# yanyan-li/PlanarSLAM

Measured on NVIDIA H100. Metric: rgbd_frames_per_sec_640x480, higher is better.
Workload: dtype u8/f64

## Files before the change

planarslam_b200/csrc/lsd_kernels.cuh:

```cuda
#pragma once
#include <cuda_runtime.h>

#include <cfloat>
#include <cstdint>

#include "lsd_detsincos.h"
#include "lsd_rectenum.h"
#include "pslam_internal.h"

namespace pslam {

struct LsdGeom {
    int w, h;
    int W, H;
    int refine;
    int seg_cap;
    int cand_cap;
    int r2r_staged;
    int rect_enum;
    int min_reg_size;
    double rho, prec, p, log_nt, density_th, log_eps;
    const double* lgamma_tab;
};
#define LSD_LGAMMA_N 8192

#define LSD_ANG_UNDEF 0x7f800000u
#define LSD_ANG_USED 0x80000000u

#define LSD_PI 3.14159265358979323846
#define LSD_DEG2RAD (LSD_PI / 180)
#define LSD_3_2_PI ((3 * LSD_PI) / 2)
#define LSD_2PI (2 * LSD_PI)
#define LSD_LN10 2.30258509299404568402

__device__ __forceinline__ float lsd_fast_atan2_deg(float y, float x) {
    const float p1 = 0.9997878412794807f * (float)(180 / 3.14159265358979323846);
    const float p3 = -0.3258083974640975f * (float)(180 / 3.14159265358979323846);
    const float p5 = 0.1555786518463281f * (float)(180 / 3.14159265358979323846);
    const float p7 = -0.04432655554792128f * (float)(180 / 3.14159265358979323846);
    const float ax = fabsf(x), ay = fabsf(y);
    const bool wide = ax >= ay;
    const float num = wide ? ay : ax, den = __fadd_rn(wide ? ax : ay, (float)DBL_EPSILON);
    const float c = __fdiv_rn(num, den);
    const float c2 = __fmul_rn(c, c);
    float a = __fmul_rn(__fadd_rn(__fmul_rn(__fadd_rn(__fmul_rn(__fadd_rn(__fmul_rn(p7, c2), p5), c2), p3), c2), p1), c);
    if (!wide) a = __fsub_rn(90.f, a);
    if (x < 0) a = __fsub_rn(180.f, a);
    if (y < 0) a = __fsub_rn(360.f, a);
    return a;
}
__device__ __forceinline__ double lsd_angle(int gx, int gy) { return (double)lsd_fast_atan2_deg((float)gx, (float)(-gy)) * LSD_DEG2RAD; }
__device__ __forceinline__ double lsd_norm(int gx, int gy) { return sqrt((double)(gx * gx + gy * gy) / 4.0); }

template <int V>
__device__ __noinline__ void lsd_sincos(double x, double& s, double& c) { lsd_sincos_body(x, s, c); }

#define LSD_TW 64
#define LSD_TH 16
#define LSD_SW 88
#define LSD_SH 28
__global__ void __launch_bounds__(256) k_lsd_blur_scale(LsdGeom g, const uint8_t* __restrict__ gray, const int16_t* __restrict__ ix,
                                                        const int16_t* __restrict__ ax, const int16_t* __restrict__ iy, const int16_t* __restrict__ ay,
                                                        uint8_t* __restrict__ scaled) {
    __shared__ uint8_t s_src[LSD_SH][LSD_SW];
    __shared__ uint16_t s_h[LSD_SH][LSD_SW];
    __shared__ uint8_t s_b[LSD_SH][LSD_SW];
    const int frame = blockIdx.z, X0 = blockIdx.x * LSD_TW, Y0 = blockIdx.y * LSD_TH;
    const int X1 = min(X0 + LSD_TW, g.W) - 1, Y1 = min(Y0 + LSD_TH, g.H) - 1;
    const int bx0 = ix[X0], bx1 = min(ix[X1] + 1, g.w - 1), by0 = iy[Y0], by1 = min(iy[Y1] + 1, g.h - 1);
    const int sx0 = bx0 - 2, sy0 = by0 - 2, sw = bx1 - bx0 + 5, sh = by1 - by0 + 5;
    const uint8_t* src = gray + (size_t)frame * g.w * g.h;
// ... 61 lines not shown

__global__ void __launch_bounds__(256) k_lsd_gradient4(LsdGeom g, const uint8_t* __restrict__ scaled, const float2* __restrict__ cs_lut,
                                                       uint32_t* __restrict__ ang, float2* __restrict__ cs_out, uint32_t* __restrict__ gxy, int32_t* __restrict__ smax) {
    const int frame = blockIdx.z;
    const int W4 = g.W >> 2;
    const int xq = blockIdx.x * 64 + (threadIdx.x & 63), y = blockIdx.y * 4 + (threadIdx.x >> 6);
    const bool inside = xq < W4 && y < g.H;
    const uint8_t* s = scaled + (size_t)frame * g.W * g.H;
    uint32_t a_w[4] = {LSD_ANG_UNDEF, LSD_ANG_UNDEF, LSD_ANG_UNDEF, LSD_ANG_UNDEF}, g_w[4] = {0, 0, 0, 0};
    float2 cs[4];
#pragma unroll
    for (int i = 0; i < 4; ++i) cs[i] = make_float2(0.f, 0.f);
    int sq = 0;
    if (inside && y < g.H - 1) {
        const int x = xq * 4;
        const uint32_t* r0 = reinterpret_cast<const uint32_t*>(s + (size_t)y * g.W + x);
        const uint32_t* r1 = reinterpret_cast<const uint32_t*>(s + (size_t)(y + 1) * g.W + x);
        const uint32_t w0 = r0[0], w1 = r1[0];
        const bool more = x + 4 < g.W;
        const uint32_t n0 = more ? (uint32_t)s[(size_t)y * g.W + x + 4] : 0u, n1 = more ? (uint32_t)s[(size_t)(y + 1) * g.W + x + 4] : 0u;
        const uint32_t e0 = __funnelshift_r(w0, n0, 8), e1 = __funnelshift_r(w1, n1, 8);
#pragma unroll
        for (int i = 0; i < 4; ++i) {
            if (x + i >= g.W - 1) continue;
            const int pa = (w0 >> (8 * i)) & 255, pb = (e0 >> (8 * i)) & 255, pc = (w1 >> (8 * i)) & 255, pd = (e1 >> (8 * i)) & 255;
            const int DA = pd - pa, BC = pb - pc;
            const int gx = DA + BC, gy = DA - BC;
            g_w[i] = ((uint32_t)gx & 0xffffu) | ((uint32_t)gy << 16);
            if (lsd_norm(gx, gy) > g.rho) {
                sq = max(sq, gx * gx + gy * gy); a_w[i] = __float_as_uint(lsd_fast_atan2_deg((float)gx, (float)(-gy)));
                cs[i] = __ldg(cs_lut + (gx + 510) * 1021 + (gy + 510));
            }
        }
    }
    if (inside) {
        const size_t o = (size_t)frame * g.W * g.H + (size_t)y * g.W + (size_t)xq * 4;
        *reinterpret_cast<uint4*>(ang + o) = make_uint4(a_w[0], a_w[1], a_w[2], a_w[3]);
        *reinterpret_cast<uint4*>(gxy + o) = make_uint4(g_w[0], g_w[1], g_w[2], g_w[3]);
        float4* co = reinterpret_cast<float4*>(cs_out + o);
        co[0] = make_float4(cs[0].x, cs[0].y, cs[1].x, cs[1].y);
        co[1] = make_float4(cs[2].x, cs[2].y, cs[3].x, cs[3].y);
    }
    for (int o = 16; o; o >>= 1) sq = max(sq, __shfl_xor_sync(0xffffffffu, sq, o));
    if ((threadIdx.x & 31) == 0 && sq > 0) atomicMax(&smax[frame], sq);
}

struct LsdRect { double x1, y1, x2, y2, width, x, y, theta, dx, dy, prec, p; };

#define LSD_RING 64
struct LsdFrame {
    uint32_t* ang;
    const float2* cs; const uint32_t* gxy;
    uint32_t* reg; uint32_t* order;
    uint32_t* ring;
    int W, H;
};
__device__ __forceinline__ bool lsd_word_used(uint32_t w) { return (w & LSD_ANG_USED) != 0; }
__device__ __forceinline__ bool lsd_word_defined(uint32_t w) { return (w & 0x7fffffffu) < LSD_ANG_UNDEF; }
__device__ __forceinline__ float lsd_word_deg(uint32_t w) { return __uint_as_float(w & 0x7fffffffu); }
__device__ __forceinline__ double lsd_word_angle(uint32_t w) { return (double)lsd_word_deg(w) * LSD_DEG2RAD; }
__device__ __forceinline__ double lsd_pix_norm(const LsdFrame& F, int x, int y) {
    const uint32_t v = __ldg(F.gxy + (size_t)y * F.W + x);
    return lsd_norm((int)(short)(v & 0xffff), (int)(short)(v >> 16));
}

__device__ __forceinline__ bool lsd_aligned_angle(double a, double theta, double prec) {
    double n_theta = theta - a;
    if (n_theta < 0) n_theta = -n_theta;
    if (n_theta > LSD_3_2_PI) {
        n_theta -= LSD_2PI;
        if (n_theta < 0) n_theta = -n_theta;
    }
    return n_theta <= prec;
}

__device__ __forceinline__ double lsd_angle_diff_signed(double a, double b) {
    double diff = a - b;
    while (diff <= -LSD_PI) diff += LSD_2PI;
    while (diff > LSD_PI) diff -= LSD_2PI;
    return diff;
}
__device__ __forceinline__ bool lsd_double_equal(double a, double b) {
    if (a == b) return true;
    const double abs_diff = fabs(a - b), aa = fabs(a), bb = fabs(b);
    double abs_max = (aa > bb) ? aa : bb;
    if (abs_max < DBL_MIN) abs_max = DBL_MIN;
    return (abs_diff / abs_max) <= (100.0 * DBL_EPSILON);
}
__device__ __forceinline__ double lsd_dist_sq(double x1, double y1, double x2, double y2) { return (x2 - x1) * (x2 - x1) + (y2 - y1) * (y2 - y1); }

__device__ __forceinline__ uint32_t lsd_reg_read(const LsdFrame& F, int idx, int size) {
    return size - idx <= LSD_RING ? F.ring[idx & (LSD_RING - 1)] : F.reg[idx];
}
template <int V>
__device__ __noinline__ int lsd_region_grow(const LsdFrame& F, const LsdGeom& g, uint32_t seed, double prec, double& reg_angle_out) {
    const int lane = threadIdx.x & 31;
    const int q = lane >> 3, k8 = lane & 7;
    const int kk = k8 + (k8 >= 4);
    const int dyl = kk / 3 - 1, dxl = kk % 3 - 1;
    const int sx = seed & 0xffff, sy = seed >> 16;
    const uint32_t ws = F.ang[(size_t)sy * F.W + sx];
    double reg_angle = lsd_word_angle(ws);
    const double seed_angle = reg_angle;
    float sumdx = 0.f, sumdy = 0.f;
    if (lane == 0) { F.reg[0] = seed; F.ring[0] = seed; F.ang[(size_t)sy * F.W + sx] = ws | LSD_ANG_USED; }
    __syncwarp();
    int size = 1, i = 0;
    bool have_next = false;
    uint32_t np_next = 0xffffffffu, w_next = LSD_ANG_UNDEF;
    while (true) {
        const int navail = min(4, size - i);
        uint32_t npix, w;
        if (have_next) { npix = np_next; w = w_next; }
        else {
            npix = 0xffffffffu; w = LSD_ANG_UNDEF;
            if (q < navail) {
                const uint32_t pp = lsd_reg_read(F, i + q, size);
                const int nx = (int)(pp & 0xffff) + dxl, ny = (int)(pp >> 16) + dyl;
                if (nx >= 0 && ny >= 0 && nx < F.W && ny < F.H) { w = F.ang[(size_t)ny * F.W + nx]; npix = (uint32_t)nx | ((uint32_t)ny << 16); }
            }
        }
        have_next = size - i >= 8;
        np_next = 0xffffffffu; w_next = LSD_ANG_UNDEF;
        if (have_next) {
            const uint32_t pp = lsd_reg_read(F, i + 4 + q, size);
            const int nx = (int)(pp & 0xffff) + dxl, ny = (int)(pp >> 16) + dyl;
            if (nx >= 0 && ny >= 0 && nx < F.W && ny < F.H) { w_next = F.ang[(size_t)ny * F.W + nx]; np_next = (uint32_t)nx | ((uint32_t)ny << 16); }
        }
        bool cand = lsd_word_defined(w) && !lsd_word_used(w);
        const double a_n = lsd_word_angle(w);
        float2 csv = make_float2(0.f, 0.f);
        bool have_cs = cand && lsd_aligned_angle(a_n, reg_angle, prec);
        if (have_cs) csv = __ldg(F.cs + (size_t)(npix >> 16) * F.W + (npix & 0xffff));
        int last = -1;
        while (true) {
            const bool al = cand && lane > last && lsd_aligned_angle(a_n, reg_angle, prec);
            const unsigned m = __ballot_sync(0xffffffffu, al);
            if (!m) break;
            const int j = __ffs(m) - 1;
            if (lane == j) {
                if (!have_cs) { csv = __ldg(F.cs + (size_t)(npix >> 16) * F.W + (npix & 0xffff)); have_cs = true; }
                F.ang[(size_t)(npix >> 16) * F.W + (npix & 0xffff)] = w | LSD_ANG_USED;
                F.reg[size] = npix; F.ring[size & (LSD_RING - 1)] = npix;
            }
            const float cj = __shfl_sync(0xffffffffu, csv.x, j), sj = __shfl_sync(0xffffffffu, csv.y, j);
            const uint32_t np = __shfl_sync(0xffffffffu, npix, j);
            if (size == 1) { double sn0, cs0; lsd_sincos<V>(seed_angle, sn0, cs0); sumdx = (float)cs0; sumdy = (float)sn0; }
            sumdx = __fadd_rn(sumdx, cj);
            sumdy = __fadd_rn(sumdy, sj);
            reg_angle = (double)lsd_fast_atan2_deg(sumdy, sumdx) * LSD_DEG2RAD;
            if (npix == np) cand = false;
            if (np_next == np) w_next |= LSD_ANG_USED;
            ++size;
            last = j;
        }
        __syncwarp();
        i += navail;
        if (i >= size) break;
    }
    reg_angle_out = reg_angle;
    return size;
}

template <int V>
__device__ __noinline__ void lsd_region2rect_shfl(const LsdFrame& F, int size, double reg_angle, double prec, double p, LsdRect& rec) {
    const int lane = threadIdx.x & 31;
    double x = 0, y = 0, sum = 0;
    for (int base = 0; base < size; base += 32) {
        int mx = 0, my = 0; double mw = 0;
        if (base + lane < size) {
            const uint32_t pp = F.reg[base + lane];
            mx = pp & 0xffff; my = pp >> 16;
            mw = lsd_pix_norm(F, mx, my);
        }
        const int cnt = min(32, size - base);
        for (int t = 0; t < cnt; ++t) {
            const double w = __shfl_sync(0xffffffffu, mw, t);
            const int px = __shfl_sync(0xffffffffu, mx, t), py = __shfl_sync(0xffffffffu, my, t);
            x += (double)px * w;
            y += (double)py * w;
            sum += w;
        }
    }
    x /= sum;
    y /= sum;
    double Ixx = 0.0, Iyy = 0.0, Ixy = 0.0;
    for (int base = 0; base < size; base += 32) {
        int mx = 0, my = 0; double mw = 0;
        if (base + lane < size) {
            const uint32_t pp = F.reg[base + lane];
            mx = pp & 0xffff; my = pp >> 16;
            mw = lsd_pix_norm(F, mx, my);
        }
        const int cnt = min(32, size - base);
        for (int t = 0; t < cnt; ++t) {
            const double w = __shfl_sync(0xffffffffu, mw, t);
            const double ddx = (double)__shfl_sync(0xffffffffu, mx, t) - x, ddy = (double)__shfl_sync(0xffffffffu, my, t) - y;
            Ixx += ddy * ddy * w;
            Iyy += ddx * ddx * w;
            Ixy -= ddx * ddy * w;
        }
    }
    const double lambda = 0.5 * (Ixx + Iyy - sqrt((Ixx - Iyy) * (Ixx - Iyy) + 4.0 * Ixy * Ixy));
    double theta = (fabs(Ixx) > fabs(Iyy)) ? (double)lsd_fast_atan2_deg((float)(lambda - Ixx), (float)Ixy) : (double)lsd_fast_atan2_deg((float)Ixy, (float)(lambda - Iyy));
    theta *= LSD_DEG2RAD;
    if (fabs(lsd_angle_diff_signed(theta, reg_angle)) > prec) theta += LSD_PI;
    double dx, dy;
    lsd_sincos<V>(theta, dy, dx);
    double l_min = 0, l_max = 0, w_min = 0, w_max = 0;
    for (int base = 0; base < size; base += 32) {
        int mx = 0, my = 0;
        if (base + lane < size) { const uint32_t pp = F.reg[base + lane]; mx = pp & 0xffff; my = pp >> 16; }
        const int cnt = min(32, size - base);
        for (int t = 0; t < cnt; ++t) {
            const double regdx = (double)__shfl_sync(0xffffffffu, mx, t) - x, regdy = (double)__shfl_sync(0xffffffffu, my, t) - y;
            const double l = regdx * dx + regdy * dy;
            const double w = -regdx * dy + regdy * dx;
            if (l > l_max) l_max = l; else if (l < l_min) l_min = l;
            if (w > w_max) w_max = w; else if (w < w_min) w_min = w;
        }
    }
    rec.x1 = x + l_min * dx; rec.y1 = y + l_min * dy;
    rec.x2 = x + l_max * dx; rec.y2 = y + l_max * dy;
    rec.width = w_max - w_min;
    rec.x = x; rec.y = y; rec.theta = theta; rec.dx = dx; rec.dy = dy; rec.prec = prec; rec.p = p;
    if (rec.width < 1.0) rec.width = 1.0;
}

template <int V>
__device__ __noinline__ void lsd_region2rect(const LsdFrame& F, const LsdGeom& g, int size, double reg_angle, double prec, double p, LsdRect& rec) {
    if (!g.r2r_staged) { lsd_region2rect_shfl<V>(F, size, reg_angle, prec, p, rec); return; }
    __shared__ double s_stage[96];
    const int lane = threadIdx.x & 31;
    const double* const mine = s_stage + 32 * (lane < 3 ? lane : 2);
    double acc = 0;
    for (int base = 0; base < size; base += 32) {
        if (base + lane < size) {
            const uint32_t pp = F.reg[base + lane];
            const int mx = pp & 0xffff, my = pp >> 16;
            const double mw = lsd_pix_norm(F, mx, my);
            s_stage[lane] = (double)mx * mw; s_stage[32 + lane] = (double)my * mw; s_stage[64 + lane] = mw;
        }
        __syncwarp();
        const int cnt = min(32, size - base);
        for (int t = 0; t < cnt; ++t) acc += mine[t];
        __syncwarp();
    }
    const double sum = __shfl_sync(0xffffffffu, acc, 2);
    const double x = __shfl_sync(0xffffffffu, acc, 0) / sum, y = __shfl_sync(0xffffffffu, acc, 1) / sum;
    acc = 0;
    for (int base = 0; base < size; base += 32) {
        if (base + lane < size) {
            const uint32_t pp = F.reg[base + lane];
            const int mx = pp & 0xffff, my = pp >> 16;
            const double mw = lsd_pix_norm(F, mx, my);
            const double ddx = (double)mx - x, ddy = (double)my - y;
            s_stage[lane] = ddy * ddy * mw; s_stage[32 + lane] = ddx * ddx * mw; s_stage[64 + lane] = -(ddx * ddy * mw);
        }
        __syncwarp();
        const int cnt = min(32, size - base);
        for (int t = 0; t < cnt; ++t) acc += mine[t];
        __syncwarp();
    }
    const double Ixx = __shfl_sync(0xffffffffu, acc, 0), Iyy = __shfl_sync(0xffffffffu, acc, 1), Ixy = __shfl_sync(0xffffffffu, acc, 2);
    const double lambda = 0.5 * (Ixx + Iyy - sqrt((Ixx - Iyy) * (Ixx - Iyy) + 4.0 * Ixy * Ixy));
    double theta = (fabs(Ixx) > fabs(Iyy)) ? (double)lsd_fast_atan2_deg((float)(lambda - Ixx), (float)Ixy) : (double)lsd_fast_atan2_deg((float)Ixy, (float)(lambda - Iyy));
    theta *= LSD_DEG2RAD;
    if (fabs(lsd_angle_diff_signed(theta, reg_angle)) > prec) theta += LSD_PI;
    double dx, dy;
    lsd_sincos<V>(theta, dy, dx);
    double l_min = 0, l_max = 0, w_min = 0, w_max = 0;
    for (int i = lane; i < size; i += 32) {
        const uint32_t pp = F.reg[i];
        const double regdx = (double)(pp & 0xffff) - x, regdy = (double)(pp >> 16) - y;
        const double l = regdx * dx + regdy * dy;
        const double w = -regdx * dy + regdy * dx;
        if (l > l_max) l_max = l; else if (l < l_min) l_min = l;
        if (w > w_max) w_max = w; else if (w < w_min) w_min = w;
    }
#pragma unroll
    for (int o = 16; o; o >>= 1) {
        const double a = __shfl_xor_sync(0xffffffffu, l_max, o), b = __shfl_xor_sync(0xffffffffu, l_min, o);
        const double c = __shfl_xor_sync(0xffffffffu, w_max, o), d = __shfl_xor_sync(0xffffffffu, w_min, o);
        if (a > l_max) l_max = a;
        if (b < l_min) l_min = b;
        if (c > w_max) w_max = c;
        if (d < w_min) w_min = d;
    }
    rec.x1 = x + l_min * dx; rec.y1 = y + l_min * dy;
    rec.x2 = x + l_max * dx; rec.y2 = y + l_max * dy;
    rec.width = w_max - w_min;
    rec.x = x; rec.y = y; rec.theta = theta; rec.dx = dx; rec.dy = dy; rec.prec = prec; rec.p = p;
    if (rec.width < 1.0) rec.width = 1.0;
}

__device__ __forceinline__ double lsd_density(int size, const LsdRect& rec) {
    return (double)size / (sqrt(lsd_dist_sq(rec.x1, rec.y1, rec.x2, rec.y2)) * rec.width);
}

template <int V>
__device__ __noinline__ bool lsd_refine(const LsdFrame& F, const LsdGeom& g, int& size, double& reg_angle, LsdRect& rec) {
    const int lane = threadIdx.x & 31;
    double density = lsd_density(size, rec);
    if (density >= g.density_th) return true;
    const uint32_t p0 = F.reg[0];
    const double xc = (double)(p0 & 0xffff), yc = (double)(p0 >> 16);
    const double ang_c = lsd_word_angle(F.ang[(size_t)(p0 >> 16) * F.W + (p0 & 0xffff)]);
    double sum = 0, s_sum = 0;
    int n = 0;
    for (int base = 0; base < size; base += 32) {
        int mx = 0, my = 0; double ma = 0;
        if (base + lane < size) {
            const uint32_t pp = F.reg[base + lane];
            mx = pp & 0xffff; my = pp >> 16;
            const uint32_t wv = F.ang[(size_t)my * F.W + mx];
            F.ang[(size_t)my * F.W + mx] = wv & 0x7fffffffu;
            ma = lsd_word_angle(wv);
        }
        const int cnt = min(32, size - base);
        for (int t = 0; t < cnt; ++t) {
            const double a = __shfl_sync(0xffffffffu, ma, t);
            const double px = (double)__shfl_sync(0xffffffffu, mx, t), py = (double)__shfl_sync(0xffffffffu, my, t);
            if (sqrt(lsd_dist_sq(xc, yc, px, py)) < rec.width) {
                const double ang_d = lsd_angle_diff_signed(a, ang_c);
                sum += ang_d;
                s_sum += ang_d * ang_d;
                ++n;
            }
        }
    }
    __syncwarp();
    const double mean_angle = sum / (double)n;
    const double tau = 2.0 * sqrt((s_sum - 2.0 * mean_angle * sum) / (double)n + mean_angle * mean_angle);
    size = lsd_region_grow<V>(F, g, p0, tau, reg_angle);
    if (size < 2) return false;
    lsd_region2rect<V>(F, g, size, reg_angle, g.prec, g.p, rec);
    density = lsd_density(size, rec);
    if (density >= g.density_th) return true;
    double radSq1 = lsd_dist_sq(xc, yc, rec.x1, rec.y1), radSq2 = lsd_dist_sq(xc, yc, rec.x2, rec.y2);
    double radSq = radSq1 > radSq2 ? radSq1 : radSq2;
    while (density < g.density_th) {
        radSq *= 0.75 * 0.75;
        for (int i = 0; i < size; ++i) {
            const uint32_t pp = F.reg[i];
            const double px = (double)(pp & 0xffff), py = (double)(pp >> 16);
            if (lsd_dist_sq(xc, yc, px, py) > radSq) {
                const uint32_t lastp = F.reg[size - 1];
                __syncwarp();
                if (lane == 0) { F.ang[(size_t)(pp >> 16) * F.W + (pp & 0xffff)] &= 0x7fffffffu; F.reg[i] = lastp; F.reg[size - 1] = pp; }
                __syncwarp();
                --size;
                --i;
            }
        }
        if (size < 2) return false;
        lsd_region2rect<V>(F, g, size, reg_angle, g.prec, g.p, rec);
        density = lsd_density(size, rec);
    }
    return true;
}

__device__ __forceinline__ double lsd_log_gamma1(double x) {
    if (x > 15.0) return 0.918938533204673 + (x - 0.5) * log(x) - x + 0.5 * x * log(x * sinh(1 / x) + 1 / (810.0 * pow(x, 6.0)));
    const double q[7] = {75122.6331530, 80916.6278952, 36308.2951477, 8687.24529705, 1168.92649479, 83.8676043424, 2.50662827511};
    double a = (x + 0.5) * log(x + 5.5) - (x + 5.5);
    double b = 0;
    for (int n = 0; n < 7; ++n) {
        a -= log(x + (double)n);
        b += q[n] * pow(x, (double)n);
    }
    return a + log(b);
}
__device__ __noinline__ double lsd_nfa_scalar(int n, int k, double p, double log_nt, const double* __restrict__ lgamma_tab) {
    if (n == 0 || k == 0) return -log_nt;
    if (n == k) return -log_nt - (double)n * log10(p);
    const double p_term = p / (1 - p);
    double lg0, lg1, lg2;
    if (n + 1 < LSD_LGAMMA_N) { lg0 = __ldg(lgamma_tab + n + 1); lg1 = __ldg(lgamma_tab + k + 1); lg2 = __ldg(lgamma_tab + n - k + 1); }
    else { lg0 = lsd_log_gamma1((double)n + 1); lg1 = lsd_log_gamma1((double)k + 1); lg2 = lsd_log_gamma1((double)(n - k) + 1); }
    const double log1term = lg0 - lg1 - lg2 + (double)k * log(p) + (double)(n - k) * log(1.0 - p);
    double term = exp(log1term);
    if (lsd_double_equal(term, 0)) {
        if (k > n * p) return -log1term / LSD_LN10 - log_nt;
        return -log_nt;
    }
    double bin_tail = term;
    const double tolerance = 0.1;
    for (int i = k + 1; i <= n; ++i) {
        const double bin_term = (double)(n - i + 1) / (double)i;
        const double mult_term = bin_term * p_term;
        term *= mult_term;
        bin_tail += term;
        if (bin_term < 1) {
            const double err = term * ((1 - pow(mult_term, (double)(n - i + 1))) / (1 - mult_term) - 1);
            if (err < tolerance * fabs(-log10(bin_tail) - log_nt) * bin_tail) break;
        }
    }
    return -log10(bin_tail) - log_nt;
}

__device__ __forceinline__ double lsd_inter_low(double x, double x1, double y1, double x2, double y2) {
    if (lsd_double_equal(x1, x2) && y1 < y2) return y1;
    if (lsd_double_equal(x1, x2) && y1 > y2) return y2;
    return y1 + (x - x1) * (y2 - y1) / (x2 - x1);
}
__device__ __forceinline__ double lsd_inter_hi(double x, double x1, double y1, double x2, double y2) {
    if (lsd_double_equal(x1, x2) && y1 < y2) return y2;
    if (lsd_double_equal(x1, x2) && y1 > y2) return y1;
    return y1 + (x - x1) * (y2 - y1) / (x2 - x1);
// ... 143 lines not shown
    const int t0 = wid * per, t1 = min(n_scan, t0 + per);
    uint32_t* cnt = s_cnt + wid * 1024;
    for (int base = t0; base < t1; base += 32) {
        const int t = base + lane;
        int bin = -1;
        if (t < t1) { const int y = t / Wm, x = t - y * Wm; bin = lsd_order_bin(s, g.W, x, y, g.rho, bin_coef); }
        const unsigned peers = __match_any_sync(0xffffffffu, bin);
        if (bin >= 0 && lane == __ffs(peers) - 1) cnt[bin] += __popc(peers);
        __syncwarp();
    }
    __syncthreads();
    {
        const int rb = 1023 - tid;
        uint32_t tot = 0;
        for (int w = 0; w < 32; ++w) tot += s_cnt[w * 1024 + rb];
        uint32_t incl = tot;
        for (int o = 1; o < 32; o <<= 1) { const uint32_t v = __shfl_up_sync(0xffffffffu, incl, o); if (lane >= o) incl += v; }
        if (lane == 31) s_wsum[wid] = incl;
        __syncthreads();
        if (wid == 0) {
            uint32_t v = s_wsum[lane], iv = v;
            for (int o = 1; o < 32; o <<= 1) { const uint32_t u = __shfl_up_sync(0xffffffffu, iv, o); if (lane >= o) iv += u; }
            s_wsum[lane] = iv - v;
            if (lane == 31) n_order[frame] = (int32_t)iv;
        }
        __syncthreads();
        uint32_t run = s_wsum[wid] + incl - tot;
        for (int w = 0; w < 32; ++w) { const uint32_t c = s_cnt[w * 1024 + rb]; s_cnt[w * 1024 + rb] = run; run += c; }
        (void)s_tot;
    }
    __syncthreads();
    for (int base = t0; base < t1; base += 32) {
        const int t = base + lane;
        int bin = -1; uint32_t pix = 0;
        if (t < t1) { const int y = t / Wm, x = t - y * Wm; bin = lsd_order_bin(s, g.W, x, y, g.rho, bin_coef); pix = (uint32_t)x | ((uint32_t)y << 16); }
        const unsigned peers = __match_any_sync(0xffffffffu, bin);
        if (bin >= 0) {
            const int rank = __popc(peers & ((1u << lane) - 1u));
            const int leader = __ffs(peers) - 1;
            uint32_t basep = 0;
            if (lane == leader) { basep = cnt[bin]; cnt[bin] = basep + __popc(peers); }
            basep = __shfl_sync(peers, basep, leader);
            order[basep + rank] = pix;
        }
        __syncwarp();
    }
}

template <int V>
__global__ void __launch_bounds__(32, V) k_lsd_regions(LsdGeom g, int nframes, uint32_t* __restrict__ ang_all, const float2* __restrict__ cs_all, const uint32_t* __restrict__ gxy_all,
                                                    const int32_t* __restrict__ smax, uint32_t* __restrict__ reg_all, const uint32_t* __restrict__ order_all,
                                                    const int32_t* __restrict__ n_order, double* __restrict__ cands, int32_t* __restrict__ n_cand,
                                                    int32_t* __restrict__ status) {
    __shared__ uint32_t s_ring[LSD_RING];
    const int lane = threadIdx.x & 31;
    const int frame = blockIdx.x;
    if (frame >= nframes) return;
    const size_t npx = (size_t)g.W * g.H;
    LsdFrame F;
    F.ang = ang_all + (size_t)frame * npx; F.cs = cs_all + (size_t)frame * npx; F.gxy = gxy_all + (size_t)frame * npx; F.reg = reg_all + (size_t)frame * npx;
    F.order = const_cast<uint32_t*>(order_all) + (size_t)frame * npx; F.W = g.W; F.H = g.H;
    F.ring = s_ring;
    int count_out = 0;
    const int n_def = smax[frame] > 0 ? n_order[frame] : 0;
    {
        for (int base = 0; base < n_def; base += 32) {
            const uint32_t mypix = base + lane < n_def ? F.order[base + lane] : 0u;
            int last = -1;
            while (true) {
                bool fresh = false;
                if (base + lane < n_def && lane > last) fresh = !lsd_word_used(F.ang[(size_t)(mypix >> 16) * F.W + (mypix & 0xffff)]);
                const unsigned m = __ballot_sync(0xffffffffu, fresh);
                if (!m) break;
                const int j = __ffs(m) - 1;
                last = j;
                const uint32_t seed = __shfl_sync(0xffffffffu, mypix, j);
                double reg_angle;
                int size = lsd_region_grow<V>(F, g, seed, g.prec, reg_angle);
                if (size < g.min_reg_size) continue;
                LsdRect rc;
                lsd_region2rect<V>(F, g, size, reg_angle, g.prec, g.p, rc);
                if (g.refine > 0 && !lsd_refine<V>(F, g, size, reg_angle, rc)) continue;
                if (count_out < g.cand_cap && lane < 12) {
                    const double v = lane == 0 ? rc.x1 : lane == 1 ? rc.y1 : lane == 2 ? rc.x2 : lane == 3 ? rc.y2 : lane == 4 ? rc.width : lane == 5 ? rc.x :
                                     lane == 6 ? rc.y : lane == 7 ? rc.theta : lane == 8 ? rc.dx : lane == 9 ? rc.dy : lane == 10 ? rc.prec : rc.p;
                    cands[((size_t)frame * g.cand_cap + count_out) * 12 + lane] = v;
                }
                ++count_out;
            }
        }
    }
    if (lane == 0) {
        n_cand[frame] = count_out;
        status[frame] = count_out > g.cand_cap ? 1 : 0;
    }
}

__device__ __forceinline__ void lsd_load_cand(const double* __restrict__ c, LsdRect& rc) {
    rc.x1 = c[0]; rc.y1 = c[1]; rc.x2 = c[2]; rc.y2 = c[3]; rc.width = c[4]; rc.x = c[5]; rc.y = c[6]; rc.theta = c[7]; rc.dx = c[8]; rc.dy = c[9];
    rc.prec = c[10]; rc.p = c[11];
}
__global__ void __launch_bounds__(64) k_lsd_validate(LsdGeom g, const uint32_t* __restrict__ ang_all, const double* __restrict__ cands, const int32_t* __restrict__ n_cand,
                                                     double* __restrict__ cand_nfa, uint32_t* __restrict__ fail_list, int32_t* __restrict__ n_fail) {
    const int frame = blockIdx.y;
    const int ci = blockIdx.x * 64 + threadIdx.x;
    const int n = min(n_cand[frame], g.cand_cap);
    if (ci >= n) return;
    LsdFrame F;
    F.ang = const_cast<uint32_t*>(ang_all) + (size_t)frame * g.W * g.H; F.cs = nullptr; F.gxy = nullptr; F.reg = nullptr; F.order = nullptr; F.ring = nullptr; F.W = g.W; F.H = g.H;
    LsdRect rc;
    lsd_load_cand(cands + ((size_t)frame * g.cand_cap + ci) * 12, rc);
    const double log_nfa = lsd_rect_nfa_scalar(F, g, rc);
    cand_nfa[(size_t)frame * g.cand_cap + ci] = log_nfa;
    if (!(log_nfa > g.log_eps)) fail_list[(size_t)frame * g.cand_cap + atomicAdd(&n_fail[frame], 1)] = (uint32_t)ci;
}
__global__ void __launch_bounds__(64) k_lsd_improve(LsdGeom g, const uint32_t* __restrict__ ang_all, double* __restrict__ cands, double* __restrict__ cand_nfa,
                                                    const uint32_t* __restrict__ fail_list, const int32_t* __restrict__ n_fail) {
    const int frame = blockIdx.y;
    const int k = blockIdx.x * 64 + threadIdx.x;
    if (k >= n_fail[frame]) return;
    const int ci = (int)fail_list[(size_t)frame * g.cand_cap + k];
    LsdFrame F;
    F.ang = const_cast<uint32_t*>(ang_all) + (size_t)frame * g.W * g.H; F.cs = nullptr; F.gxy = nullptr; F.reg = nullptr; F.order = nullptr; F.ring = nullptr; F.W = g.W; F.H = g.H;
    double* c = cands + ((size_t)frame * g.cand_cap + ci) * 12;
    LsdRect rc;
    lsd_load_cand(c, rc);
    const double log_nfa = lsd_rect_improve_rest(F, g, rc, cand_nfa[(size_t)frame * g.cand_cap + ci]);
    c[0] = rc.x1; c[1] = rc.y1; c[2] = rc.x2; c[3] = rc.y2; c[4] = rc.width; c[11] = rc.p;
    cand_nfa[(size_t)frame * g.cand_cap + ci] = log_nfa;
}

__global__ void __launch_bounds__(256) k_lsd_emit(LsdGeom g, const double* __restrict__ cands, const int32_t* __restrict__ n_cand, const double* __restrict__ cand_nfa,
                                                  float4* __restrict__ segs, double* __restrict__ wpn, int32_t* __restrict__ n_segs, int32_t* __restrict__ status) {
    __shared__ int s_warp[8];
    __shared__ int s_base;
    const int frame = blockIdx.x, tid = threadIdx.x, lane = tid & 31, wid = tid >> 5;
    const int n = min(n_cand[frame], g.cand_cap);
    if (tid == 0) s_base = 0;
    __syncthreads();
    for (int c0 = 0; c0 < n; c0 += 256) {
        const int ci = c0 + tid;
        bool keep = false;
        double nfa = -1;
        if (ci < n) {
            if (g.refine >= 2) { nfa = cand_nfa[(size_t)frame * g.cand_cap + ci]; keep = nfa > g.log_eps; }
            else keep = true;
        }
        const unsigned m = __ballot_sync(0xffffffffu, keep);
        if (lane == 0) s_warp[wid] = __popc(m);
        __syncthreads();
        int off = s_base;
        for (int w = 0; w < wid; ++w) off += s_warp[w];
        const int slot = off + __popc(m & ((1u << lane) - 1u));
        if (keep && slot < g.seg_cap) {
            const double* c = cands + ((size_t)frame * g.cand_cap + ci) * 12;
            double x1 = c[0], y1 = c[1], x2 = c[2], y2 = c[3], width = c[4];
            x1 += 0.5; y1 += 0.5; x2 += 0.5; y2 += 0.5;
            x1 /= 0.8; y1 /= 0.8; x2 /= 0.8; y2 /= 0.8; width /= 0.8;
            segs[(size_t)frame * g.seg_cap + slot] = make_float4((float)x1, (float)y1, (float)x2, (float)y2);
            double* o = wpn + ((size_t)frame * g.seg_cap + slot) * 3;
            o[0] = width; o[1] = c[11]; o[2] = nfa;
        }
        __syncthreads();
        if (tid == 0) { int t = 0; for (int w = 0; w < 8; ++w) t += s_warp[w]; s_base += t; }
        __syncthreads();
    }
    if (tid == 0) {
        n_segs[frame] = s_base;
        if (s_base > g.seg_cap) status[frame] |= 2;
    }
}

struct LsdKeyLine {
    float angle; int32_t class_id; int32_t octave; float pt_x, pt_y; float response; float size;
    float startPointX, startPointY, endPointX, endPointY, sPointInOctaveX, sPointInOctaveY, ePointInOctaveX, ePointInOctaveY;
    float lineLength; int32_t numOfPixels;
// ... 52 lines not shown
```

planarslam_b200/csrc/lsd_pipeline.cu:

```cuda
#include <algorithm>
#include <cfloat>
#include <cmath>
#include <cstring>
#include <cstdlib>
#include <string>

#include "lsd_kernels.cuh"
#include "lbd_kernels.cuh"

namespace pslam {

struct LsdBuffers {
    LsdGeom g;
    int max_batch = 0, last_n = 0, max_lines_cap = 0;
    int16_t *d_ix = nullptr, *d_ax = nullptr, *d_iy = nullptr, *d_ay = nullptr;
    float2* d_lut = nullptr; double* d_lgamma = nullptr;
    uint8_t* d_gray = nullptr;
    uint8_t* d_scaled = nullptr; uint32_t* d_ang = nullptr; float2* d_cs = nullptr; uint32_t* d_gxy = nullptr; int32_t* d_smax = nullptr;
    uint32_t* d_reg = nullptr; uint32_t* d_order = nullptr; int32_t* d_norder = nullptr;
    double* d_cands = nullptr; double* d_cand_nfa = nullptr; int32_t* d_ncand = nullptr;
    uint32_t* d_fail = nullptr; int32_t* d_nfail = nullptr;
    float4* d_segs = nullptr; double* d_wpn = nullptr; int32_t* d_nsegs = nullptr; int32_t* d_status = nullptr;
    LsdKeyLine* d_kl = nullptr; double* d_lf = nullptr; int32_t* d_nkl = nullptr;
    int16_t *d_dx = nullptr, *d_dy = nullptr; float *d_glocal = nullptr, *d_gglobal = nullptr; uint8_t* d_ldesc = nullptr; float* d_lbd72 = nullptr;
    std::vector<int32_t> h_n, h_status;
};

static int lsd_cv_round(double v) { return (int)std::nearbyint(v); }

static float host_fast_atan2_deg(float y, float x) {
    const float p1 = 0.9997878412794807f * (float)(180 / 3.14159265358979323846);
    const float p3 = -0.3258083974640975f * (float)(180 / 3.14159265358979323846);
    const float p5 = 0.1555786518463281f * (float)(180 / 3.14159265358979323846);
    const float p7 = -0.04432655554792128f * (float)(180 / 3.14159265358979323846);
    const float ax = std::fabs(x), ay = std::fabs(y);
    float a, c, c2;
    if (ax >= ay) { c = ay / (ax + (float)DBL_EPSILON); c2 = c * c; a = (((p7 * c2 + p5) * c2 + p3) * c2 + p1) * c; }
    else { c = ax / (ay + (float)DBL_EPSILON); c2 = c * c; a = 90.f - (((p7 * c2 + p5) * c2 + p3) * c2 + p1) * c; }
    if (x < 0) a = 180.f - a;
    if (y < 0) a = 360.f - a;
    return a;
}

static const int LSD_SEG_CAP = 4096;
#define LSD_REGIONS_OCC 24

int lsd_alloc(pslam_ctx* c) {
    if (c->lsd) return PSLAM_OK;
    LsdBuffers* Bp = new LsdBuffers();
    LsdBuffers& B = *Bp;
    LsdGeom& g = B.g;
    g.w = c->cfg.width; g.h = c->cfg.height;
    const double SCALE = 0.8, ANG_TH = 22.5, QUANT = 2.0;
    g.W = lsd_cv_round(g.w * SCALE); g.H = lsd_cv_round(g.h * SCALE);
    if (g.W < 8 || g.H < 8 || g.W > 32767 || g.H > 32767) { delete Bp; return set_error(c, PSLAM_E_INVALID, "image size unsupported by the line-segment detector"); }
    g.refine = 2;
    g.seg_cap = g.cand_cap = std::max(LSD_SEG_CAP, (int)(((long long)LSD_SEG_CAP * g.w * g.h / (640 * 480) + 1023) / 1024 * 1024));
    {
        const char* e = std::getenv("PSLAM_LSD_RECT_ENUM");
        g.rect_enum = (e && (!std::strcmp(e, "published") || !std::strcmp(e, "0"))) ? 0 : 1;
        { const char* r = std::getenv("PSLAM_LSD_R2R"); g.r2r_staged = (r && (!std::strcmp(r, "shfl") || !std::strcmp(r, "0"))) ? 0 : 1; }
    }
    g.prec = LSD_PI * ANG_TH / 180; g.p = ANG_TH / 180; g.rho = QUANT / std::sin(g.prec);
    g.log_nt = 5 * (std::log10(double(g.W)) + std::log10(double(g.H))) / 2 + std::log10(11.0);
    g.min_reg_size = (int)(size_t)(-g.log_nt / std::log10(g.p));
    g.density_th = 0.7; g.log_eps = 0;
    B.max_batch = c->cfg.max_batch;
    auto coef = [SCALE](int dn, int sn, std::vector<int16_t>& idx, std::vector<int16_t>& a) {
        idx.resize(dn); a.resize(dn);
        const double scale = 1.0 / SCALE;
        for (int d = 0; d < dn; ++d) {
            const double f = (d + 0.5) * scale - 0.5;
            int i = (int)std::floor(f);
            double fr = f - i;
            if (i < 0) { i = 0; fr = 0; }
            if (i >= sn - 1) { i = sn - 1; fr = 0; }
            idx[d] = (int16_t)i; a[d] = (int16_t)std::floor(fr * 256 + 0.5);
        }
    };
    std::vector<int16_t> ix, ax, iy, ay;
    coef(g.W, g.w, ix, ax); coef(g.H, g.h, iy, ay);
    for (int X0 = 0; X0 < g.W; X0 += LSD_TW) {
        const int X1 = std::min(X0 + LSD_TW, g.W) - 1;
        if (std::min(ix[X1] + 1, g.w - 1) - ix[X0] + 5 > LSD_SW) { delete Bp; return set_error(c, PSLAM_E_INVALID, "LSD tile bound (width)"); }
    }
    for (int Y0 = 0; Y0 < g.H; Y0 += LSD_TH) {
        const int Y1 = std::min(Y0 + LSD_TH, g.H) - 1;
        if (std::min(iy[Y1] + 1, g.h - 1) - iy[Y0] + 5 > LSD_SH) { delete Bp; return set_error(c, PSLAM_E_INVALID, "LSD tile bound (height)"); }
    }
    std::vector<float2> lut((size_t)1021 * 1021);
    for (int gx = -510; gx <= 510; ++gx)
        for (int gy = -510; gy <= 510; ++gy) {
            const double ang = (double)host_fast_atan2_deg((float)gx, (float)(-gy)) * LSD_DEG2RAD;
            const float af = (float)ang;
            lut[(size_t)(gx + 510) * 1021 + (gy + 510)] = make_float2(std::cos(af), std::sin(af));
        }
    std::vector<double> lgam(LSD_LGAMMA_N, 0.0);
    for (int i = 1; i < LSD_LGAMMA_N; ++i) {
        const double x = (double)i;
        if (x > 15.0) lgam[i] = 0.918938533204673 + (x - 0.5) * std::log(x) - x + 0.5 * x * std::log(x * std::sinh(1 / x) + 1 / (810.0 * std::pow(x, 6.0)));
        else {
            static const double q[7] = {75122.6331530, 80916.6278952, 36308.2951477, 8687.24529705, 1168.92649479, 83.8676043424, 2.50662827511};
            double a = (x + 0.5) * std::log(x + 5.5) - (x + 5.5), b = 0;
            for (int n = 0; n < 7; ++n) { a -= std::log(x + double(n)); b += q[n] * std::pow(x, double(n)); }
            lgam[i] = a + std::log(b);
        }
    }
    const size_t npx = (size_t)g.W * g.H, nb = (size_t)B.max_batch;
#define LA(ptr, bytes) do { const int rc_ = check_cuda(c, cudaMalloc((void**)&(ptr), (bytes)), "cudaMalloc(lsd)"); if (rc_ != PSLAM_OK) { c->lsd = Bp; lsd_free(c); return rc_; } } while (0)
    LA(B.d_ix, g.W * 2); LA(B.d_ax, g.W * 2); LA(B.d_iy, g.H * 2); LA(B.d_ay, g.H * 2); LA(B.d_lut, lut.size() * sizeof(float2)); LA(B.d_lgamma, LSD_LGAMMA_N * 8);
    LA(B.d_gray, nb * g.w * g.h); LA(B.d_scaled, nb * npx); LA(B.d_ang, nb * npx * 4); LA(B.d_cs, nb * npx * 8); LA(B.d_gxy, nb * npx * 4); LA(B.d_smax, nb * 4);
    LA(B.d_reg, nb * npx * 4); LA(B.d_order, nb * npx * 4); LA(B.d_norder, nb * 4);
    LA(B.d_fail, nb * g.cand_cap * 4); LA(B.d_nfail, nb * 4);
    LA(B.d_cands, nb * g.cand_cap * 12 * 8); LA(B.d_cand_nfa, nb * g.cand_cap * 8); LA(B.d_ncand, nb * 4);
// ... 267 lines not shown
```

Before: 5183.

## Batch region-grow writes, prefetch cos/sin, and warp-parallelize refine compaction

Region growing now loads the cos/sin pair together with the angle word during neighbour probing. It records the accepted lanes in a mask and writes all accepted pixels after the serial ballot loop, using popcount offsets, instead of one lane storing inside each iteration. Refine replaces the serial per-pixel shuffle loops with per-lane computation plus shared-memory reduction. Its pixel-removal loop becomes a warp-parallel ballot compaction in place of a serial swap with a warp sync per removed pixel. The unused shuffle region2rect path, its environment toggle and the ring pointer are removed, and the ring buffer moves into the grow function. This adds unconditional cs loads for unaligned neighbours, and it changes the order in which the sum and removals are computed, which may alter results slightly.

```diff
diff --git a/planarslam_b200/csrc/lsd_kernels.cuh b/planarslam_b200/csrc/lsd_kernels.cuh
--- a/planarslam_b200/csrc/lsd_kernels.cuh
+++ b/planarslam_b200/csrc/lsd_kernels.cuh
@@ -16,7 +16,6 @@
     int refine;
     int seg_cap;
     int cand_cap;
-    int r2r_staged;
     int rect_enum;
     int min_reg_size;
     double rho, prec, p, log_nt, density_th, log_eps;
@@ -184,7 +183,6 @@
     uint32_t* ang;
     const float2* cs; const uint32_t* gxy;
     uint32_t* reg; uint32_t* order;
-    uint32_t* ring;
     int W, H;
 };
 __device__ __forceinline__ bool lsd_word_used(uint32_t w) { return (w & LSD_ANG_USED) != 0; }
@@ -221,147 +219,81 @@
 }
 __device__ __forceinline__ double lsd_dist_sq(double x1, double y1, double x2, double y2) { return (x2 - x1) * (x2 - x1) + (y2 - y1) * (y2 - y1); }
 
-__device__ __forceinline__ uint32_t lsd_reg_read(const LsdFrame& F, int idx, int size) {
-    return size - idx <= LSD_RING ? F.ring[idx & (LSD_RING - 1)] : F.reg[idx];
-}
+struct LsdGrown { double angle; int size; };
 template <int V>
-__device__ __noinline__ int lsd_region_grow(const LsdFrame& F, const LsdGeom& g, uint32_t seed, double prec, double& reg_angle_out) {
+__device__ __noinline__ LsdGrown lsd_region_grow(uint32_t* ang, const float2* __restrict__ cs, uint32_t* reg, int W, int H, uint32_t seed, double prec) {
+    __shared__ uint32_t ring[LSD_RING];
     const int lane = threadIdx.x & 31;
+    const unsigned below = (1u << lane) - 1u;
     const int q = lane >> 3, k8 = lane & 7;
     const int kk = k8 + (k8 >= 4);
     const int dyl = kk / 3 - 1, dxl = kk % 3 - 1;
     const int sx = seed & 0xffff, sy = seed >> 16;
-    const uint32_t ws = F.ang[(size_t)sy * F.W + sx];
+    const uint32_t ws = ang[(size_t)sy * W + sx];
     double reg_angle = lsd_word_angle(ws);
-    const double seed_angle = reg_angle;
     float sumdx = 0.f, sumdy = 0.f;
-    if (lane == 0) { F.reg[0] = seed; F.ring[0] = seed; F.ang[(size_t)sy * F.W + sx] = ws | LSD_ANG_USED; }
+    if (lane == 0) { reg[0] = seed; ring[0] = seed; ang[(size_t)sy * W + sx] = ws | LSD_ANG_USED; }
     __syncwarp();
+    auto probe = [&](int idx, int size, uint32_t& npix, uint32_t& w, float2& csv) {
+        const uint32_t pp = size - idx <= LSD_RING ? ring[idx & (LSD_RING - 1)] : reg[idx];
+        const int nx = (int)(pp & 0xffff) + dxl, ny = (int)(pp >> 16) + dyl;
+        if (nx >= 0 && ny >= 0 && nx < W && ny < H) {
+            const size_t o = (size_t)ny * W + nx;
+            w = ang[o]; csv = __ldg(cs + o); npix = (uint32_t)nx | ((uint32_t)ny << 16);
+        }
+    };
     int size = 1, i = 0;
     bool have_next = false;
     uint32_t np_next = 0xffffffffu, w_next = LSD_ANG_UNDEF;
+    float2 cs_next = make_float2(0.f, 0.f);
     while (true) {
         const int navail = min(4, size - i);
-        uint32_t npix, w;
-        if (have_next) { npix = np_next; w = w_next; }
-        else {
-            npix = 0xffffffffu; w = LSD_ANG_UNDEF;
-            if (q < navail) {
-                const uint32_t pp = lsd_reg_read(F, i + q, size);
-                const int nx = (int)(pp & 0xffff) + dxl, ny = (int)(pp >> 16) + dyl;
-                if (nx >= 0 && ny >= 0 && nx < F.W && ny < F.H) { w = F.ang[(size_t)ny * F.W + nx]; npix = (uint32_t)nx | ((uint32_t)ny << 16); }
-            }
-        }
+        uint32_t npix = 0xffffffffu, w = LSD_ANG_UNDEF;
+        float2 csv = make_float2(0.f, 0.f);
+        if (have_next) { npix = np_next; w = w_next; csv = cs_next; }
+        else if (q < navail) probe(i + q, size, npix, w, csv);
         have_next = size - i >= 8;
-        np_next = 0xffffffffu; w_next = LSD_ANG_UNDEF;
-        if (have_next) {
-            const uint32_t pp = lsd_reg_read(F, i + 4 + q, size);
-            const int nx = (int)(pp & 0xffff) + dxl, ny = (int)(pp >> 16) + dyl;
-            if (nx >= 0 && ny >= 0 && nx < F.W && ny < F.H) { w_next = F.ang[(size_t)ny * F.W + nx]; np_next = (uint32_t)nx | ((uint32_t)ny << 16); }
-        }
+        np_next = 0xffffffffu; w_next = LSD_ANG_UNDEF; cs_next = make_float2(0.f, 0.f);
+        if (have_next) probe(i + 4 + q, size, np_next, w_next, cs_next);
         bool cand = lsd_word_defined(w) && !lsd_word_used(w);
         const double a_n = lsd_word_angle(w);
-        float2 csv = make_float2(0.f, 0.f);
-        bool have_cs = cand && lsd_aligned_angle(a_n, reg_angle, prec);
-        if (have_cs) csv = __ldg(F.cs + (size_t)(npix >> 16) * F.W + (npix & 0xffff));
+        if (size == 1 && __any_sync(0xffffffffu, cand && lsd_aligned_angle(a_n, reg_angle, prec))) {
+            double sn0, cs0;
+            lsd_sincos<V>(reg_angle, sn0, cs0);
+            sumdx = (float)cs0; sumdy = (float)sn0;
+        }
         int last = -1;
+        unsigned taken = 0;
         while (true) {
             const bool al = cand && lane > last && lsd_aligned_angle(a_n, reg_angle, prec);
             const unsigned m = __ballot_sync(0xffffffffu, al);
             if (!m) break;
             const int j = __ffs(m) - 1;
-            if (lane == j) {
-                if (!have_cs) { csv = __ldg(F.cs + (size_t)(npix >> 16) * F.W + (npix & 0xffff)); have_cs = true; }
-                F.ang[(size_t)(npix >> 16) * F.W + (npix & 0xffff)] = w | LSD_ANG_USED;
-                F.reg[size] = npix; F.ring[size & (LSD_RING - 1)] = npix;
-            }
             const float cj = __shfl_sync(0xffffffffu, csv.x, j), sj = __shfl_sync(0xffffffffu, csv.y, j);
             const uint32_t np = __shfl_sync(0xffffffffu, npix, j);
-            if (size == 1) { double sn0, cs0; lsd_sincos<V>(seed_angle, sn0, cs0); sumdx = (float)cs0; sumdy = (float)sn0; }
             sumdx = __fadd_rn(sumdx, cj);
             sumdy = __fadd_rn(sumdy, sj);
             reg_angle = (double)lsd_fast_atan2_deg(sumdy, sumdx) * LSD_DEG2RAD;
             if (npix == np) cand = false;
             if (np_next == np) w_next |= LSD_ANG_USED;
-            ++size;
+            taken |= 1u << j;
             last = j;
         }
+        if (taken >> lane & 1u) {
+            const int at = size + __popc(taken & below);
+            ang[(size_t)(npix >> 16) * W + (npix & 0xffff)] = w | LSD_ANG_USED;
+            reg[at] = npix; ring[at & (LSD_RING - 1)] = npix;
+        }
+        size += __popc(taken);
         __syncwarp();
         i += navail;
         if (i >= size) break;
     }
-    reg_angle_out = reg_angle;
-    return size;
+    return {reg_angle, size};
 }
 
 template <int V>
-__device__ __noinline__ void lsd_region2rect_shfl(const LsdFrame& F, int size, double reg_angle, double prec, double p, LsdRect& rec) {
-    const int lane = threadIdx.x & 31;
-    double x = 0, y = 0, sum = 0;
-    for (int base = 0; base < size; base += 32) {
-        int mx = 0, my = 0; double mw = 0;
-        if (base + lane < size) {
-            const uint32_t pp = F.reg[base + lane];
-            mx = pp & 0xffff; my = pp >> 16;
-            mw = lsd_pix_norm(F, mx, my);
-        }
-        const int cnt = min(32, size - base);
-        for (int t = 0; t < cnt; ++t) {
-            const double w = __shfl_sync(0xffffffffu, mw, t);
-            const int px = __shfl_sync(0xffffffffu, mx, t), py = __shfl_sync(0xffffffffu, my, t);
-            x += (double)px * w;
-            y += (double)py * w;
-            sum += w;
-        }
-    }
-    x /= sum;
-    y /= sum;
-    double Ixx = 0.0, Iyy = 0.0, Ixy = 0.0;
-    for (int base = 0; base < size; base += 32) {
-        int mx = 0, my = 0; double mw = 0;
-        if (base + lane < size) {
-            const uint32_t pp = F.reg[base + lane];
-            mx = pp & 0xffff; my = pp >> 16;
-            mw = lsd_pix_norm(F, mx, my);
-        }
-        const int cnt = min(32, size - base);
-        for (int t = 0; t < cnt; ++t) {
-            const double w = __shfl_sync(0xffffffffu, mw, t);
-            const double ddx = (double)__shfl_sync(0xffffffffu, mx, t) - x, ddy = (double)__shfl_sync(0xffffffffu, my, t) - y;
-            Ixx += ddy * ddy * w;
-            Iyy += ddx * ddx * w;
-            Ixy -= ddx * ddy * w;
-        }
-    }
-    const double lambda = 0.5 * (Ixx + Iyy - sqrt((Ixx - Iyy) * (Ixx - Iyy) + 4.0 * Ixy * Ixy));
-    double theta = (fabs(Ixx) > fabs(Iyy)) ? (double)lsd_fast_atan2_deg((float)(lambda - Ixx), (float)Ixy) : (double)lsd_fast_atan2_deg((float)Ixy, (float)(lambda - Iyy));
-    theta *= LSD_DEG2RAD;
-    if (fabs(lsd_angle_diff_signed(theta, reg_angle)) > prec) theta += LSD_PI;
-    double dx, dy;
-    lsd_sincos<V>(theta, dy, dx);
-    double l_min = 0, l_max = 0, w_min = 0, w_max = 0;
-    for (int base = 0; base < size; base += 32) {
-        int mx = 0, my = 0;
-        if (base + lane < size) { const uint32_t pp = F.reg[base + lane]; mx = pp & 0xffff; my = pp >> 16; }
-        const int cnt = min(32, size - base);
-        for (int t = 0; t < cnt; ++t) {
-            const double regdx = (double)__shfl_sync(0xffffffffu, mx, t) - x, regdy = (double)__shfl_sync(0xffffffffu, my, t) - y;
-            const double l = regdx * dx + regdy * dy;
-            const double w = -regdx * dy + regdy * dx;
-            if (l > l_max) l_max = l; else if (l < l_min) l_min = l;
-            if (w > w_max) w_max = w; else if (w < w_min) w_min = w;
-        }
-    }
-    rec.x1 = x + l_min * dx; rec.y1 = y + l_min * dy;
-    rec.x2 = x + l_max * dx; rec.y2 = y + l_max * dy;
-    rec.width = w_max - w_min;
-    rec.x = x; rec.y = y; rec.theta = theta; rec.dx = dx; rec.dy = dy; rec.prec = prec; rec.p = p;
-    if (rec.width < 1.0) rec.width = 1.0;
-}
-
-template <int V>
-__device__ __noinline__ void lsd_region2rect(const LsdFrame& F, const LsdGeom& g, int size, double reg_angle, double prec, double p, LsdRect& rec) {
-    if (!g.r2r_staged) { lsd_region2rect_shfl<V>(F, size, reg_angle, prec, p, rec); return; }
+__device__ __noinline__ void lsd_region2rect(const LsdFrame& F, int size, double reg_angle, double prec, double p, LsdRect& rec) {
     __shared__ double s_stage[96];
     const int lane = threadIdx.x & 31;
     const double* const mine = s_stage + 32 * (lane < 3 ? lane : 2);
@@ -432,61 +364,86 @@
 
 template <int V>
 __device__ __noinline__ bool lsd_refine(const LsdFrame& F, const LsdGeom& g, int& size, double& reg_angle, LsdRect& rec) {
+    __shared__ double s_ang[64];
     const int lane = threadIdx.x & 31;
+    const unsigned below = (1u << lane) - 1u;
     double density = lsd_density(size, rec);
     if (density >= g.density_th) return true;
-    const uint32_t p0 = F.reg[0];
+    uint32_t* const ang = F.ang;
+    uint32_t* const reg = F.reg;
+    const int W = F.W;
+    const uint32_t p0 = reg[0];
     const double xc = (double)(p0 & 0xffff), yc = (double)(p0 >> 16);
-    const double ang_c = lsd_word_angle(F.ang[(size_t)(p0 >> 16) * F.W + (p0 & 0xffff)]);
-    double sum = 0, s_sum = 0;
+    const double ang_c = lsd_word_angle(ang[(size_t)(p0 >> 16) * W + (p0 & 0xffff)]);
+    const double* const mine = s_ang + 32 * (lane & 1);
+    double acc = 0;
     int n = 0;
     for (int base = 0; base < size; base += 32) {
-        int mx = 0, my = 0; double ma = 0;
+        bool near = false;
         if (base + lane < size) {
-            const uint32_t pp = F.reg[base + lane];
-            mx = pp & 0xffff; my = pp >> 16;
-            const uint32_t wv = F.ang[(size_t)my * F.W + mx];
-            F.ang[(size_t)my * F.W + mx] = wv & 0x7fffffffu;
-            ma = lsd_word_angle(wv);
-        }
+            const uint32_t pp = reg[base + lane];
+            const int mx = pp & 0xffff, my = pp >> 16;
+            const uint32_t wv = ang[(size_t)my * W + mx];
+            ang[(size_t)my * W + mx] = wv & 0x7fffffffu;
+            double ang_d = 0;
+            near = sqrt(lsd_dist_sq(xc, yc, (double)mx, (double)my)) < rec.width;
+            if (near) ang_d = lsd_angle_diff_signed(lsd_word_angle(wv), ang_c);
+            s_ang[lane] = ang_d; s_ang[32 + lane] = ang_d * ang_d;
+        }
+        n += __popc(__ballot_sync(0xffffffffu, near));
+        __syncwarp();
         const int cnt = min(32, size - base);
-        for (int t = 0; t < cnt; ++t) {
-            const double a = __shfl_sync(0xffffffffu, ma, t);
-            const double px = (double)__shfl_sync(0xffffffffu, mx, t), py = (double)__shfl_sync(0xffffffffu, my, t);
-            if (sqrt(lsd_dist_sq(xc, yc, px, py)) < rec.width) {
-                const double ang_d = lsd_angle_diff_signed(a, ang_c);
-                sum += ang_d;
-                s_sum += ang_d * ang_d;
-                ++n;
-            }
-        }
-    }
-    __syncwarp();
+        for (int t = 0; t < cnt; ++t) acc += mine[t];
+        __syncwarp();
+    }
+    const double sum = __shfl_sync(0xffffffffu, acc, 0), s_sum = __shfl_sync(0xffffffffu, acc, 1);
     const double mean_angle = sum / (double)n;
     const double tau = 2.0 * sqrt((s_sum - 2.0 * mean_angle * sum) / (double)n + mean_angle * mean_angle);
-    size = lsd_region_grow<V>(F, g, p0, tau, reg_angle);
+    const LsdGrown gr = lsd_region_grow<V>(ang, F.cs, reg, W, F.H, p0, tau);
+    size = gr.size; reg_angle = gr.angle;
     if (size < 2) return false;
-    lsd_region2rect<V>(F, g, size, reg_angle, g.prec, g.p, rec);
+    lsd_region2rect<V>(F, size, reg_angle, g.prec, g.p, rec);
     density = lsd_density(size, rec);
     if (density >= g.density_th) return true;
     double radSq1 = lsd_dist_sq(xc, yc, rec.x1, rec.y1), radSq2 = lsd_dist_sq(xc, yc, rec.x2, rec.y2);
     double radSq = radSq1 > radSq2 ? radSq1 : radSq2;
     while (density < g.density_th) {
         radSq *= 0.75 * 0.75;
-        for (int i = 0; i < size; ++i) {
-            const uint32_t pp = F.reg[i];
-            const double px = (double)(pp & 0xffff), py = (double)(pp >> 16);
-            if (lsd_dist_sq(xc, yc, px, py) > radSq) {
-                const uint32_t lastp = F.reg[size - 1];
-                __syncwarp();
-                if (lane == 0) { F.ang[(size_t)(pp >> 16) * F.W + (pp & 0xffff)] &= 0x7fffffffu; F.reg[i] = lastp; F.reg[size - 1] = pp; }
-                __syncwarp();
-                --size;
-                --i;
+        auto far_point = [&](uint32_t pp) { return lsd_dist_sq(xc, yc, (double)(pp & 0xffff), (double)(pp >> 16)) > radSq; };
+        int nfar = 0;
+        for (int base = 0; base < size; base += 32) {
+            bool f = false;
+            if (base + lane < size) {
+                const uint32_t pp = reg[base + lane];
+                f = far_point(pp);
+                if (f) ang[(size_t)(pp >> 16) * W + (pp & 0xffff)] &= 0x7fffffffu;
             }
-        }
+            nfar += __popc(__ballot_sync(0xffffffffu, f));
+        }
+        const int m = size - nfar;
+        int r = 0;
+        for (int top = size - 1; top >= m; top -= 32) {
+            const int idx = top - lane;
+            uint32_t pp = 0;
+            bool keep = false;
+            if (idx >= m) { pp = reg[idx]; keep = !far_point(pp); }
+            const unsigned k = __ballot_sync(0xffffffffu, keep);
+            if (keep) reg[size - 1 - (r + __popc(k & below))] = pp;
+            r += __popc(k);
+        }
+        __syncwarp();
+        r = 0;
+        for (int base = 0; base < m; base += 32) {
+            const int idx = base + lane;
+            const bool hole = idx < m && far_point(reg[idx]);
+            const unsigned h = __ballot_sync(0xffffffffu, hole);
+            if (hole) reg[idx] = reg[size - 1 - (r + __popc(h & below))];
+            r += __popc(h);
+        }
+        __syncwarp();
+        size = m;
         if (size < 2) return false;
-        lsd_region2rect<V>(F, g, size, reg_angle, g.prec, g.p, rec);
+        lsd_region2rect<V>(F, size, reg_angle, g.prec, g.p, rec);
         density = lsd_density(size, rec);
     }
     return true;
@@ -736,7 +693,6 @@
                                                     const int32_t* __restrict__ smax, uint32_t* __restrict__ reg_all, const uint32_t* __restrict__ order_all,
                                                     const int32_t* __restrict__ n_order, double* __restrict__ cands, int32_t* __restrict__ n_cand,
                                                     int32_t* __restrict__ status) {
-    __shared__ uint32_t s_ring[LSD_RING];
     const int lane = threadIdx.x & 31;
     const int frame = blockIdx.x;
     if (frame >= nframes) return;
@@ -744,7 +700,6 @@
     LsdFrame F;
     F.ang = ang_all + (size_t)frame * npx; F.cs = cs_all + (size_t)frame * npx; F.gxy = gxy_all + (size_t)frame * npx; F.reg = reg_all + (size_t)frame * npx;
     F.order = const_cast<uint32_t*>(order_all) + (size_t)frame * npx; F.W = g.W; F.H = g.H;
-    F.ring = s_ring;
     int count_out = 0;
     const int n_def = smax[frame] > 0 ? n_order[frame] : 0;
     {
@@ -759,11 +714,12 @@
                 const int j = __ffs(m) - 1;
                 last = j;
                 const uint32_t seed = __shfl_sync(0xffffffffu, mypix, j);
-                double reg_angle;
-                int size = lsd_region_grow<V>(F, g, seed, g.prec, reg_angle);
+                const LsdGrown gr = lsd_region_grow<V>(F.ang, F.cs, F.reg, F.W, F.H, seed, g.prec);
+                int size = gr.size;
+                double reg_angle = gr.angle;
                 if (size < g.min_reg_size) continue;
                 LsdRect rc;
-                lsd_region2rect<V>(F, g, size, reg_angle, g.prec, g.p, rc);
+                lsd_region2rect<V>(F, size, reg_angle, g.prec, g.p, rc);
                 if (g.refine > 0 && !lsd_refine<V>(F, g, size, reg_angle, rc)) continue;
                 if (count_out < g.cand_cap && lane < 12) {
                     const double v = lane == 0 ? rc.x1 : lane == 1 ? rc.y1 : lane == 2 ? rc.x2 : lane == 3 ? rc.y2 : lane == 4 ? rc.width : lane == 5 ? rc.x :
@@ -791,7 +747,7 @@
     const int n = min(n_cand[frame], g.cand_cap);
     if (ci >= n) return;
     LsdFrame F;
-    F.ang = const_cast<uint32_t*>(ang_all) + (size_t)frame * g.W * g.H; F.cs = nullptr; F.gxy = nullptr; F.reg = nullptr; F.order = nullptr; F.ring = nullptr; F.W = g.W; F.H = g.H;
+    F.ang = const_cast<uint32_t*>(ang_all) + (size_t)frame * g.W * g.H; F.cs = nullptr; F.gxy = nullptr; F.reg = nullptr; F.order = nullptr; F.W = g.W; F.H = g.H;
     LsdRect rc;
     lsd_load_cand(cands + ((size_t)frame * g.cand_cap + ci) * 12, rc);
     const double log_nfa = lsd_rect_nfa_scalar(F, g, rc);
@@ -805,7 +761,7 @@
     if (k >= n_fail[frame]) return;
     const int ci = (int)fail_list[(size_t)frame * g.cand_cap + k];
     LsdFrame F;
-    F.ang = const_cast<uint32_t*>(ang_all) + (size_t)frame * g.W * g.H; F.cs = nullptr; F.gxy = nullptr; F.reg = nullptr; F.order = nullptr; F.ring = nullptr; F.W = g.W; F.H = g.H;
+    F.ang = const_cast<uint32_t*>(ang_all) + (size_t)frame * g.W * g.H; F.cs = nullptr; F.gxy = nullptr; F.reg = nullptr; F.order = nullptr; F.W = g.W; F.H = g.H;
     double* c = cands + ((size_t)frame * g.cand_cap + ci) * 12;
     LsdRect rc;
     lsd_load_cand(c, rc);
diff --git a/planarslam_b200/csrc/lsd_pipeline.cu b/planarslam_b200/csrc/lsd_pipeline.cu
--- a/planarslam_b200/csrc/lsd_pipeline.cu
+++ b/planarslam_b200/csrc/lsd_pipeline.cu
@@ -59,7 +59,6 @@
     {
         const char* e = std::getenv("PSLAM_LSD_RECT_ENUM");
         g.rect_enum = (e && (!std::strcmp(e, "published") || !std::strcmp(e, "0"))) ? 0 : 1;
-        { const char* r = std::getenv("PSLAM_LSD_R2R"); g.r2r_staged = (r && (!std::strcmp(r, "shfl") || !std::strcmp(r, "0"))) ? 0 : 1; }
     }
     g.prec = LSD_PI * ANG_TH / 180; g.p = ANG_TH / 180; g.rho = QUANT / std::sin(g.prec);
     g.log_nt = 5 * (std::log10(double(g.W)) + std::log10(double(g.H))) / 2 + std::log10(11.0);
```

Result: faster. 5659, median of 6 (+9.2%).
